# google-research/simclr

Hardware: AMD Instinct MI355X
Metric: images/sec (whole node), ResNet-50 1x SimCLR pretraining step @224px (higher is better)
Workload: dtype f32; 1 GPU; ResNet-50 1x, 224x224, 2 views/image, per-GPU batch 512, global batch 512, NT-Xent T=0.1 + linear-eval head + LARS, global BN, dp1; global_batch=512, parallelism=dp1

## Files before the change

simclr_amd/csrc/conv.hip:

```cpp
#include "common.h"
#include <stdlib.h>
#include <string.h>
#include <mutex>
#include <type_traits>

namespace {

enum { MODE_FWD = 0, MODE_DGRAD = 1 };

struct ConvP {
  const void* x;
  const void* w;
  void* y;
  float* stats;
  int V, IH, IW, IC, OH, OW, N, KH, KW, stride, pad;
  int pixpitch;
  int M, K;
  int nslot, accumulate;
  int m_tiles, n_tiles;
  int cs, py, px, cls_h, cls_w;
  int ntaps;
  int taps[9];
  unsigned long long tap_w, dy_w, dx_w;
  const void* bn_x;
// ... 30 lines not shown
template <> struct MMA<uint16_t> {
  __device__ static __forceinline__ f32x4 run(const u32x4& a, const u32x4& b, f32x4 c) {
    return __builtin_amdgcn_mfma_f32_16x16x32_bf16(__builtin_bit_cast(bf16x8, a),
                                                   __builtin_bit_cast(bf16x8, b), c, 0, 0, 0);
  }
};
template <> struct MMA<float> {
  __device__ static __forceinline__ f32x4 run(const u32x4& a, const u32x4& b, f32x4 c) {
#pragma unroll
    for (int j = 0; j < 4; ++j)
      c = __builtin_amdgcn_mfma_f32_16x16x4f32(__uint_as_float(a[j]), __uint_as_float(b[j]), c, 0, 0, 0);
    return c;
  }
};

__device__ __forceinline__ void split_terms2(const u32x4& c0, const u32x4& c1, u32x4& hi, u32x4& lo) {
#pragma unroll
  for (int j = 0; j < 4; ++j) {
    const float x0 = __uint_as_float(j < 2 ? c0[2 * j] : c1[2 * j - 4]), x1 = __uint_as_float(j < 2 ? c0[2 * j + 1] : c1[2 * j - 3]);
    const uint32_t h = pack_bf16x2(x0, x1);
    hi[j] = h;
    lo[j] = pack_bf16x2(x0 - __uint_as_float(h << 16), x1 - __uint_as_float(h & 0xffff0000u));
  }
}
__device__ __forceinline__ void split_terms3(const u32x4& c0, const u32x4& c1, u32x4& hi, u32x4& lo, u32x4& lo2) {
#pragma unroll
  for (int j = 0; j < 4; ++j) {
    const float x0 = __uint_as_float(j < 2 ? c0[2 * j] : c1[2 * j - 4]), x1 = __uint_as_float(j < 2 ? c0[2 * j + 1] : c1[2 * j - 3]);
    const uint32_t h = pack_bf16x2(x0, x1);
    const float r0 = x0 - __uint_as_float(h << 16), r1 = x1 - __uint_as_float(h & 0xffff0000u);
    const uint32_t l = pack_bf16x2(r0, r1);
    hi[j] = h;
    lo[j] = l;
    lo2[j] = pack_bf16x2(r0 - __uint_as_float(l << 16), r1 - __uint_as_float(l & 0xffff0000u));
  }
}
__device__ __forceinline__ f32x4 mma_bf16(const u32x4& a, const u32x4& b, f32x4 c) {
  return __builtin_amdgcn_mfma_f32_16x16x32_bf16(__builtin_bit_cast(bf16x8, a), __builtin_bit_cast(bf16x8, b), c, 0, 0, 0);
}
typedef __attribute__((ext_vector_type(8))) _Float16 f16x8;
#define F16_WSCALE_LOG2 8
__device__ __forceinline__ void split_terms2_f16(const u32x4& c0, const u32x4& c1, u32x4& hi, u32x4& lo) {
#pragma unroll
  for (int j = 0; j < 4; ++j) {
    const float x0 = __uint_as_float(j < 2 ? c0[2 * j] : c1[2 * j - 4]), x1 = __uint_as_float(j < 2 ? c0[2 * j + 1] : c1[2 * j - 3]);
    uint32_t h, l;
    split_pair<true>(x0, x1, h, l);
    hi[j] = h; lo[j] = l;
  }
}
__device__ __forceinline__ f32x4 mma_f16(const u32x4& a, const u32x4& b, f32x4 c) {
  return __builtin_amdgcn_mfma_f32_16x16x32_f16(__builtin_bit_cast(f16x8, a), __builtin_bit_cast(f16x8, b), c, 0, 0, 0);
}
template <int NA, int NB, bool TR, int terms, bool PSA = false, bool PSB2 = false, typename LA, typename LB>
__device__ __forceinline__ void mma_f32_chunks(f32x4* __restrict__ accp, LA lda, LB ldb) {
  static_assert(terms == 0 || terms == 3 || terms == 6 || terms == 13, "0 = exact fp32, 3 / 6 = split-bf16 terms, 13 = three split-fp16 terms");
  static_assert(!(PSA || PSB2) || terms == 3 || terms == 13, "pre-split operand: two planes (hi, lo) = the three-term products only");
#define acc_(i, j) accp[TR ? (j) * NA + (i) : (i) * NB + (j)]
  if constexpr (terms == 0) {
#pragma unroll
    for (int ks = 0; ks < 2; ++ks) {
      u32x4 a[NA], b[NB];
#pragma unroll
      for (int i = 0; i < NA; ++i) a[i] = lda(i, ks);
#pragma unroll
      for (int j = 0; j < NB; ++j) b[j] = ldb(j, ks);
#pragma unroll
      for (int i = 0; i < NA; ++i)
#pragma unroll
        for (int j = 0; j < NB; ++j)
#pragma unroll
          for (int e = 0; e < 4; ++e)
            acc_(i, j) = __builtin_amdgcn_mfma_f32_16x16x4f32(__uint_as_float(a[i][e]), __uint_as_float(b[j][e]), acc_(i, j), 0, 0, 0);
    }
  } else if constexpr (terms == 3 || terms == 13) {
    constexpr bool F16 = terms == 13;
    auto mm = [](const u32x4& a, const u32x4& b, f32x4 c) __attribute__((always_inline)) { return F16 ? mma_f16(a, b, c) : mma_bf16(a, b, c); };
    u32x4 bh[NB], bl[NB];
#pragma unroll
    for (int j = 0; j < NB; ++j) {
      if constexpr (PSB2) { bh[j] = ldb(j, 0); bl[j] = ldb(j, 1); }
      else if constexpr (F16) split_terms2_f16(ldb(j, 0), ldb(j, 1), bh[j], bl[j]);
      else split_terms2(ldb(j, 0), ldb(j, 1), bh[j], bl[j]);
    }
#pragma unroll
    for (int i = 0; i < NA; ++i) {
      u32x4 ah, al;
      if constexpr (PSA) { ah = lda(i, 0); al = lda(i, 1); }
      else if constexpr (F16) split_terms2_f16(lda(i, 0), lda(i, 1), ah, al);
      else split_terms2(lda(i, 0), lda(i, 1), ah, al);
#pragma unroll
      for (int j = 0; j < NB; ++j) acc_(i, j) = mm(al, bh[j], acc_(i, j));
#pragma unroll
      for (int j = 0; j < NB; ++j) acc_(i, j) = mm(ah, bl[j], acc_(i, j));
#pragma unroll
      for (int j = 0; j < NB; ++j) acc_(i, j) = mm(ah, bh[j], acc_(i, j));
    }
  } else {
    u32x4 bh[NB], bl[NB], bm[NB];
#pragma unroll
    for (int j = 0; j < NB; ++j) split_terms3(ldb(j, 0), ldb(j, 1), bh[j], bl[j], bm[j]);
#pragma unroll
    for (int i = 0; i < NA; ++i) {
      u32x4 ah, al, am;
      split_terms3(lda(i, 0), lda(i, 1), ah, al, am);
#pragma unroll
      for (int j = 0; j < NB; ++j) acc_(i, j) = mma_bf16(al, bl[j], acc_(i, j));
#pragma unroll
      for (int j = 0; j < NB; ++j) acc_(i, j) = mma_bf16(am, bh[j], acc_(i, j));
#pragma unroll
      for (int j = 0; j < NB; ++j) acc_(i, j) = mma_bf16(ah, bm[j], acc_(i, j));
#pragma unroll
      for (int j = 0; j < NB; ++j) acc_(i, j) = mma_bf16(al, bh[j], acc_(i, j));
#pragma unroll
      for (int j = 0; j < NB; ++j) acc_(i, j) = mma_bf16(ah, bl[j], acc_(i, j));
#pragma unroll
      for (int j = 0; j < NB; ++j) acc_(i, j) = mma_bf16(ah, bh[j], acc_(i, j));
    }
  }
#undef acc_
}

__device__ __forceinline__ u32x4 ld16(const void* p) { return *(const u32x4*)p; }
__device__ __forceinline__ u32x4 zero16() { return (u32x4){0u, 0u, 0u, 0u}; }

__device__ __forceinline__ bool tile_of_block(int m_tiles, int n_tiles, int& mt, int& nt) {
  const int b = blockIdx.x, xcd = b & 7, idx = b >> 3;
  nt = idx % n_tiles;
  mt = (idx / n_tiles) * 8 + xcd;
  return mt < m_tiles;
// ... 227 lines not shown
    constexpr int LPR = BN * 2 / 8;
    unsigned char* Cs = smem;
    long long* rowoff = (long long*)(smem + BM * PITCH);
    if (tid < BM) rowoff[tid] = row_offset(m0 + tid);
#pragma unroll
    for (int ni = 0; ni < NI; ++ni) {
      const int nl = wn * 64 + ni * 16 + g * 4;
#pragma unroll
      for (int mi = 0; mi < MI; ++mi) {
        const int ml = wm * (MI * 16) + mi * 16 + fl;
        u32x2 pk;
        pk[0] = pack_bf16x2(acc[ni][mi][0], acc[ni][mi][1]);
        pk[1] = pack_bf16x2(acc[ni][mi][2], acc[ni][mi][3]);
        *(u32x2*)(Cs + ml * PITCH + nl * 2) = pk;
      }
    }
    __syncthreads();
    const int c8 = tid % LPR;
    const int ncol = n0 + c8 * 4;
#pragma unroll 4
    for (int r = tid / LPR; r < BM; r += 256 / LPR) {
      const long long off = rowoff[r];
      if (off >= 0 && ncol < p.N) {
        u32x2 v = *(const u32x2*)(Cs + r * PITCH + c8 * 8);
        uint16_t* dst = (uint16_t*)Y + off + ncol;
        if (p.accumulate) {
          const u32x2 o = *(const u32x2*)dst;
          v[0] = pack_bf16x2(__uint_as_float(v[0] << 16) + __uint_as_float(o[0] << 16),
                             __uint_as_float(v[0] & 0xffff0000u) + __uint_as_float(o[0] & 0xffff0000u));
          v[1] = pack_bf16x2(__uint_as_float(v[1] << 16) + __uint_as_float(o[1] << 16),
                             __uint_as_float(v[1] & 0xffff0000u) + __uint_as_float(o[1] & 0xffff0000u));
        }
        *(u32x2*)dst = v;
      }
    }
  } else {
#pragma unroll
    for (int mi = 0; mi < MI; ++mi) {
      const long long off = row_offset(m0 + wm * (MI * 16) + mi * 16 + fl);
#pragma unroll
      for (int ni = 0; ni < NI; ++ni) {
        const int n = n0 + wn * 64 + ni * 16 + g * 4;
        if (off >= 0 && n < p.N) {
          T* dst = Y + off + n;
          float v[4] = {acc[ni][mi][0], acc[ni][mi][1], acc[ni][mi][2], acc[ni][mi][3]};
          if (p.accumulate) {
#pragma unroll
            for (int r = 0; r < 4; ++r) v[r] += Elem<T>::ld(dst + r);
          }
          *(float4*)dst = make_float4(v[0], v[1], v[2], v[3]);
        }
      }
    }
  }
}

#ifndef SIMCLR_BN64_WPE
#define SIMCLR_BN64_WPE 3
#endif
template <typename T, int MODE, int BM, int BN, int NW, int STAGES, bool STATS, bool BNEPI, bool EXT = false,
          bool WIN = false, bool FAPPLY = false, int SPL = 0, bool TAIL = false, bool PSB = false, int FAS = 0, int EPS = 0, bool PSX = false>
__global__ __launch_bounds__(NW * 64, (NW == 8 || STAGES == 3) ? 1 : (BN == 64 && (sizeof(T) == 2 || SPL == 13 || (SPL == 3 && PSB))) ? SIMCLR_BN64_WPE : 2) void conv_igemm_persistent(const ConvP p) {
  static_assert(EPS == 0 || (BNEPI && EPS <= 4 && (sizeof(T) == 2 || (MODE == MODE_DGRAD && SPL == 3 && PSB && PSX && !EXT))), "EPS specialises the BNEPI epilogue");
  const int bnm = EPS ? (((EPS - 1) >> 1) ? 4 : 2) : p.bn_mode;
  const bool accu = EPS ? ((EPS - 1) & 1) != 0 : p.accumulate != 0;
  static_assert(FAS == 0 || FAPPLY, "FAS specialises the FAPPLY epilogue");
  const bool fa_res = FAS ? true : p.bn_x != nullptr;
  const bool fa_rbn = FAS ? FAS == 2 : p.bn_mean != nullptr;
  const bool fa_relu = FAS ? true : p.bn_mode != 0;
  const bool fa_mask = FAS ? true : p.bn_mask != nullptr;
  const bool fa_n32 = FAS ? true : (p.N & 31) == 0;
  static_assert(!PSB || ((SPL == 3 || SPL == 13) && sizeof(T) == 4), "pre-split weights: fp32 storage, three terms");
  static_assert(!PSX || ((SPL == 3 || SPL == 13) && sizeof(T) == 4), "pre-split gathered operand: fp32 storage, three terms");
  static_assert(SPL != 13 || PSB, "split-fp16 terms need the pre-split (scaled) weight planes");
  static_assert(!WIN || (STAGES == 2 && !EXT && NW == 4 && BM == 128 && !FAPPLY && (sizeof(T) == 2 || ((SPL == 3 || SPL == 13) && PSB))),
                "halo-window variant: 2 stages; bf16, or fp32 storage with three terms and pre-split weights");
  static_assert(!FAPPLY || (MODE == MODE_FWD && !STATS && !BNEPI && !EXT), "fused BN-apply epilogue: forward, no statistics");
  static_assert(SPL == 0 || sizeof(T) == 4, "split-bf16 terms: fp32 storage only");
  constexpr bool WPS = WIN && sizeof(T) == 4 && !PSX && (SPL == 3 || SPL == 13);
  constexpr int EPC = Elem<T>::EPC;
  constexpr int BK = 8 * EPC;
  constexpr int WN = BN / 64;
  constexpr int WM = NW / WN;
  constexpr int MI = BM / WM / 16;
  constexpr int NI = 4;
  constexpr int AJ = BM / (8 * NW);
  constexpr int BJ = BN / (8 * NW);
  static_assert(AJ >= 1 && BJ >= 1 && MI >= 1, "tile / wave configuration");
  extern __shared__ __attribute__((aligned(16))) unsigned char smem[];
  constexpr int STG = (BM + BN) * 8;
  u32x4* As = (u32x4*)smem;
  u32x4* Bs = As + BM * 8;
  u32x4* Wn = (u32x4*)smem;
  u32x4* Bw = (u32x4*)(smem + (WIN ? p.win_bytes : 0));
  float* bnp = WIN ? (float*)(Bw + 2 * BN * 8)
                   : (float*)(As + STAGES * STG);
  long long* rowoff = (long long*)(bnp + (4 + (EXT ? 1 : 0)) * BN);
  const int zrow = WIN ? (int)(((unsigned char*)(rowoff + BM) - smem) >> 7) : 0;
  constexpr bool WSUM = BM == 256;
  float2* wred = (float2*)(rowoff + BM);
  constexpr bool LDS_EPI = sizeof(T) == 2;
  constexpr int NTH = NW * 64;
  constexpr int CPR = BN / 8;
  constexpr int RPP = NTH / CPR;
  constexpr bool ROWSTATS = STATS && LDS_EPI && (BNEPI || BM == 256);
  constexpr int EH = (LDS_EPI && BM * BN * 2 > STG * 16) ? 2 : 1;
// ... 72 lines not shown
    }
  };
  const T* b_src[BJ];
  bool b_ok[BJ];
#pragma unroll
  for (int j = 0; j < BJ; ++j) {
    const int n = n0 + 8 * (wave * BJ + j) + (lane >> 3);
    b_ok[j] = n < p.N;
    b_src[j] = Wt + (long long)(b_ok[j] ? n : 0) * p.K + kc * EPC;
  }
  auto issue_tile = [&](int ti, int ci, int buf) __attribute__((always_inline)) {
    if (DIAG(2)) return;
    const int ci0 = ci * BK;
    const bool ext = EXT && ti == p.ntaps;
    const int k0 = ext ? kmain + ci0 : (int)((p.tap_w >> (4 * ti)) & 15) * p.IC + ci0;
    unsigned char* a_dst = (unsigned char*)(As + buf * STG) + wave * AJ * 1024;
    unsigned char* b_dst = (unsigned char*)(Bs + buf * STG) + wave * BJ * 1024;
#pragma unroll
    for (int j = 0; j < AJ; ++j) {
      const void* src;
      if (ext) src = a_ok[j] ? (const void*)(X2 + (long long)a_m[j] * p.pixpitch2 + kc * EPC + ci0) : p.zero;
      else src = a_tok[j] ? (const void*)(a_tp[j] + ci0) : p.zero;
      __builtin_amdgcn_global_load_lds((gptr_t)src, (lptr_t)(a_dst + j * 1024), 16, 0, 0);
    }
#pragma unroll
    for (int j = 0; j < BJ; ++j) {
      const void* src = b_ok[j] ? (const void*)(b_src[j] + k0) : p.zero;
      __builtin_amdgcn_global_load_lds((gptr_t)src, (lptr_t)(b_dst + j * 1024), 16, 0, 0);
    }
  };

  if (BNEPI || EXT || FAPPLY) {
    for (int i = tid; i < BN; i += NW * 64) {
      const int n = n0 + i;
      const bool ok = n < p.N;
      if (FAPPLY) {
        bnp[i] = ok ? p.bn_scale[n] : 0.f;
        bnp[BN + i] = ok ? p.bn_shift[n] : 0.f;
        bnp[2 * BN + i] = (ok && p.bn_mean) ? p.bn_mean[n] : 1.f;
        bnp[3 * BN + i] = (ok && p.bn_rstd) ? p.bn_rstd[n] : 0.f;
      }
      if (BNEPI) {
        bnp[i] = (ok && bnm == 2) ? p.bn_scale[n] : 0.f;
        bnp[BN + i] = (ok && bnm == 2) ? p.bn_shift[n] : 0.f;
        bnp[2 * BN + i] = (ok && p.bn_mean) ? p.bn_mean[n] : 0.f;
        bnp[3 * BN + i] = (ok && p.bn_rstd) ? p.bn_rstd[n] : 0.f;
      }
      if (EXT) bnp[4 * BN + i] = (ok && p.bias) ? p.bias[n] : 0.f;
    }
  }
  if (WSUM && STATS && LDS_EPI) {
    for (int i = lane; i < BN; i += 64) wred[wave * BN + i] = make_float2(0.f, 0.f);
  }
  const int e_cc = tid % CPR;
  float e_s[8], e_q[8];
#pragma unroll
  for (int e = 0; e < 8; ++e) { e_s[e] = 0.f; e_q[e] = 0.f; }
  float st_s[NI][4], st_q[NI][4];
  if (STATS) {
#pragma unroll
    for (int i = 0; i < NI; ++i)
#pragma unroll
      for (int r = 0; r < 4; ++r) { st_s[i][r] = 0.f; st_q[i][r] = 0.f; }
  }

  int it = 0, iti = 0, ici = 0, ibuf = 0, buf = 0;
  int issued = 0, consumed = 0;
  const int KU = WIN ? kpt : KT;
  auto part_begin = [&]() __attribute__((always_inline)) { return (part_index() * KU) / p.rem_parts; };
  auto part_end = [&]() __attribute__((always_inline)) { return ((part_index() + 1) * KU) / p.rem_parts; };
  const int part_units = has_part ? part_end() - part_begin() : 0;
  const int total = WIN ? (count * kpt + part_units) * 9 : count * KT + part_units;
  auto issue_next = [&]() __attribute__((always_inline)) {
    issue_tile(iti, ici, ibuf);
    ibuf = (ibuf + 1 == STAGES) ? 0 : ibuf + 1;
    ++issued;
    if (++ici == ((EXT && iti == p.ntaps) ? kpt2 : kpt)) {
      ici = 0;
      if (++iti == p.ntaps + ((EXT && kpt2 > 0) ? 1 : 0)) {
        iti = 0;
        ++it;
        if (it < count) setup_rows(mslot + it * mslots);
        else if (it == count && has_part) {
          setup_rows(part_tile());
          const int pka = part_begin();
          iti = pka / kpt; ici = pka - iti * kpt;
          if (EXT && iti > p.ntaps) { iti = p.ntaps; ici = pka - p.ntaps * kpt; }
        }
      }
      if (it < count + (has_part ? 1 : 0) && iti < p.ntaps) set_tap(iti);
    }
  };
  const int Wd = p.IW;
  int wti = 0, wci = (WIN && count == 0 && has_part) ? part_begin() : 0, wit = 0;
  auto issue_b = [&]() __attribute__((always_inline)) {
    const int k0 = (int)((p.tap_w >> (4 * wti)) & 15) * p.IC + wci * BK;
    unsigned char* b_dst = (unsigned char*)(Bw + ibuf * (BN * 8)) + wave * BJ * 1024;
#pragma unroll
    for (int j = 0; j < BJ; ++j) {
      const void* src = b_ok[j] ? (const void*)(b_src[j] + k0) : p.zero;
      __builtin_amdgcn_global_load_lds((gptr_t)src, (lptr_t)(b_dst + j * 1024), 16, 0, 0);
    }
    ibuf ^= 1;
    ++issued;
    if (++wti == 9) {
      wti = 0;
// ... 79 lines not shown
        win_rows(t, zr, rr);
        if constexpr (sizeof(T) == 4) {
          mma_f32_chunks<NI, MI, false, SPL, PSB, PSX || WPS>(&acc[0][0],
              [&](int i, int ks) { const int r = wn * 64 + i * 16 + fl; return Bt[r * 8 + ((ks * 4 + g) ^ (r & 7))]; },
              [&](int i, int ks) { return Wc[rr[i] * 8 + ((ks * 4 + g) ^ (rr[i] & 7))]; });
        } else {
#pragma unroll
        for (int ks = 0; ks < 2; ++ks) {
          u32x4 af[MI], bf[NI];
          win_load(Wc, rr, Bt, ks, af, bf);
          win_mma(af, bf);
        }
        }
      };
      for (int c = kt0; c < kt1; ++c) {
        __syncthreads();
        issue_win(m0w, c);
        for (int t = 0; t < 9; ++t) {
          asm volatile("s_waitcnt vmcnt(0)" ::: "memory");
          __syncthreads();
          if (issued < total) issue_b();
          if constexpr (WPS) {
            if (t == 0) {
              const int nq = p.win_j * 32 * 4;
              for (int q = tid; q < nq; q += NW * 64) {
                const int row = q >> 2, gq = q & 3;
                u32x4* w0 = Wn + row * 8 + (gq ^ (row & 7));
                u32x4* w1 = Wn + row * 8 + ((4 + gq) ^ (row & 7));
                u32x4 hi, lo;
                if constexpr (SPL == 13) split_terms2_f16(*w0, *w1, hi, lo); else split_terms2(*w0, *w1, hi, lo);
                *w0 = hi; *w1 = lo;
              }
              __syncthreads();
            }
          }
          win_step(Wn, zrow, Bw + buf * (BN * 8), t);
          buf ^= 1;
          ++consumed;
        }
      }
    } else
    for (int kt = kt0; kt < kt1; ++kt) {
      if (STAGES == 3 && issued - consumed >= 2) asm volatile("s_waitcnt vmcnt(%0)" ::"n"(AJ + BJ) : "memory");
      else asm volatile("s_waitcnt vmcnt(0)" ::: "memory");
      if (STAGES == 3) {
        asm volatile("s_waitcnt lgkmcnt(0)" ::: "memory");
        __builtin_amdgcn_s_barrier();
      } else {
        __syncthreads();
      }
      if (issued < total) issue_next();
      if constexpr (sizeof(T) == 4) {
        if (!DIAG(1))
          mma_f32_chunks<NI, MI, false, SPL, PSB, PSX>(&acc[0][0],
              [&](int i, int ks) { const int r = wn * 64 + i * 16 + fl; return Bs[buf * STG + r * 8 + ((ks * 4 + g) ^ (r & 7))]; },
              [&](int i, int ks) { const int r = wm * (MI * 16) + i * 16 + fl; return As[buf * STG + r * 8 + ((ks * 4 + g) ^ (r & 7))]; });
      } else
      if (!DIAG(1))
#pragma unroll
      for (int ks = 0; ks < 2; ++ks) {
        constexpr int MH = MI > 4 ? 4 : MI;
        u32x4 bf[NI];
#pragma unroll
        for (int i = 0; i < NI; ++i) {
          const int r = wn * 64 + i * 16 + fl;
          bf[i] = Bs[buf * STG + r * 8 + ((ks * 4 + g) ^ (r & 7))];
        }
#pragma unroll
        for (int mh = 0; mh < MI; mh += MH) {
          u32x4 af[MH];
#pragma unroll
          for (int i = 0; i < MH; ++i) {
            const int r = wm * (MI * 16) + (mh + i) * 16 + fl;
            af[i] = As[buf * STG + r * 8 + ((ks * 4 + g) ^ (r & 7))];
          }
#pragma unroll
          for (int ni = 0; ni < NI; ++ni)
#pragma unroll
            for (int mi = 0; mi < MH; ++mi) acc[ni][mh + mi] = MMA<T>::run(bf[ni], af[mi], acc[ni][mh + mi]);
        }
      }
      buf = (buf + 1 == STAGES) ? 0 : buf + 1;
      ++consumed;
    }
    if (DIAG(4)) {
      if (acc[0][0][0] == 12345.678f) Y[0] = (T)0;
      continue;
    }
    if constexpr (SPL == 13) {
#pragma unroll
      for (int i = 0; i < NI; ++i)
#pragma unroll
        for (int j = 0; j < MI; ++j) acc[i][j] *= (1.0f / (float)(1 << F16_WSCALE_LOG2));
    }
    if (part) {
      const long long slot0 = ((long long)(mslot / p.rem_parts) * p.n_tiles + nt) * (p.rem_parts - 1);
      const int pj = part_index();
      constexpr int FR = NI * MI;
      if (pj != 0) {
        const __amdgpu_buffer_rsrc_t rp = __builtin_amdgcn_make_buffer_rsrc(
            (void*)((f32x4*)p.part_ws + (slot0 + pj - 1) * (long long)(FR * NTH)), 0, FR * NTH * 16, 0x00020000);
#pragma unroll
        for (int ni = 0; ni < NI; ++ni)
#pragma unroll
          for (int mi = 0; mi < MI; ++mi)
            __builtin_amdgcn_raw_buffer_store_b128(__builtin_bit_cast(u32x4, acc[ni][mi]), rp, tid * 16, (ni * MI + mi) * NTH * 16, 16);
        asm volatile("s_waitcnt vmcnt(0)" ::: "memory");
// ... 271 lines not shown
    auto load_row = [&](int mi) __attribute__((always_inline)) {
      const bool ok = offs[mi] >= 0;
      const long long a = ok ? offs[mi] : 0;
#pragma unroll
      for (int ni = 0; ni < NI; ++ni) {
        if (EAC) pr[ni] = *(const float4*)(Y + a + ni * 16);
        if (EBM == 2) xr[ni] = *(const float4*)(bx + a + ni * 16);
      }
      if (EBM == 4) mr = *(const u32x4*)(bmk + ((a - (ok ? g * 4 : 0)) >> 2));
    };
    load_row(0);
#pragma unroll
    for (int mi = 0; mi < MI; ++mi) {
#pragma unroll
      for (int ni = 0; ni < NI; ++ni) {
        if (offs[mi] >= 0) {
          const int nl = nl0 + ni * 16;
          float v[4] = {acc[ni][mi][0], acc[ni][mi][1], acc[ni][mi][2], acc[ni][mi][3]};
          if (EAC) { v[0] += pr[ni].x; v[1] += pr[ni].y; v[2] += pr[ni].z; v[3] += pr[ni].w; }
          float xf[4] = {0.f, 0.f, 0.f, 0.f}, mk[4];
          if (EBM == 4) {
            const unsigned mbits = mr[ni] >> (8 * g);
#pragma unroll
            for (int r = 0; r < 4; ++r) mk[r] = ((mbits >> r) & 1u) ? 1.f : 0.f;
          } else {
            xf[0] = xr[ni].x; xf[1] = xr[ni].y; xf[2] = xr[ni].z; xf[3] = xr[ni].w;
            const float4 sc = *(const float4*)(bnp + nl), sh = *(const float4*)(bnp + BN + nl);
            mk[0] = fmaf(xf[0], sc.x, sh.x); mk[1] = fmaf(xf[1], sc.y, sh.y);
            mk[2] = fmaf(xf[2], sc.z, sh.z); mk[3] = fmaf(xf[3], sc.w, sh.w);
          }
          const float4 mu = *(const float4*)(bnp + 2 * BN + nl), rs = *(const float4*)(bnp + 3 * BN + nl);
          const float mua[4] = {mu.x, mu.y, mu.z, mu.w}, rsa[4] = {rs.x, rs.y, rs.z, rs.w};
#pragma unroll
          for (int r = 0; r < 4; ++r) {
#pragma clang fp contract(off)
            v[r] = mk[r] > 0.f ? v[r] : 0.f;
            st_s[ni][r] += v[r];
            st_q[ni][r] += v[r] * (xf[r] - mua[r]) * rsa[r];
            acc[ni][mi][r] = v[r];
          }
        }
        __builtin_amdgcn_sched_barrier(0);
      }
      if (mi + 1 < MI) load_row(mi + 1);
      __builtin_amdgcn_sched_barrier(0);
      if (offs[mi] >= 0) {
#pragma unroll
        for (int ni = 0; ni < NI; ++ni)
          *(float4*)(Y + offs[mi] + ni * 16) = make_float4(acc[ni][mi][0], acc[ni][mi][1], acc[ni][mi][2], acc[ni][mi][3]);
      }
    }
    } else {
    float4 pvt[NI];
    if (sizeof(T) == 4 && MODE == MODE_FWD && STATS && !BNEPI && p.pivot) {
#pragma unroll
      for (int ni = 0; ni < NI; ++ni) {
        const int n = n0 + wn * 64 + ni * 16 + g * 4;
        pvt[ni] = n < p.N ? *(const float4*)(p.pivot + n) : make_float4(0.f, 0.f, 0.f, 0.f);
      }
    }
#pragma unroll
    for (int mi = 0; mi < MI; ++mi) {
      const int m = m0 + wm * (MI * 16) + mi * 16 + fl;
      long long off = -1;
      bool prior = p.accumulate != 0;
      if (flat) {
        if (m < p.M) off = (long long)m * p.N;
        if (p.accumulate == 2) {
          const int rem = m % (p.OH * p.OW), iy = rem / p.OW, ix = rem - iy * p.OW;
          prior = ((iy | ix) & 1) == 0;
        }
      } else if (m < p.M) {
        const int v = m / cls_hw;
        const int rem = m - v * cls_hw;
        const int ca = rem / p.cls_w, cb = rem - ca * p.cls_w;
        off = (((long long)v * p.OH + ca * p.cs + p.py) * p.OW + cb * p.cs + p.px) * p.N;
        if (p.accumulate == 2) prior = (((ca * p.cs + p.py) | (cb * p.cs + p.px)) & 1) == 0;
      }
#pragma unroll
      for (int ni = 0; ni < NI; ++ni) {
        const int n = n0 + wn * 64 + ni * 16 + g * 4;
        if (STATS && !BNEPI) {
          if (sizeof(T) == 4 && MODE == MODE_FWD && p.pivot) {
            if (off >= 0 && n < p.N) {
              const float pa[4] = {pvt[ni].x, pvt[ni].y, pvt[ni].z, pvt[ni].w};
#pragma unroll
              for (int r = 0; r < 4; ++r) { const float v = acc[ni][mi][r] - pa[r]; st_s[ni][r] += v; st_q[ni][r] += v * v; }
            }
          } else {
#pragma unroll
          for (int r = 0; r < 4; ++r) { const float v = acc[ni][mi][r]; st_s[ni][r] += v; st_q[ni][r] += v * v; }
          }
        }
        if (off >= 0 && n < p.N) {
          T* dst = Y + off + n;
          float v[4] = {acc[ni][mi][0], acc[ni][mi][1], acc[ni][mi][2], acc[ni][mi][3]};
          if (EXT) {
            const float4 bi = *(const float4*)(bnp + 4 * BN + wn * 64 + ni * 16 + g * 4);
            v[0] += bi.x; v[1] += bi.y; v[2] += bi.z; v[3] += bi.w;
          }
          if (prior) {
#pragma unroll
            for (int r = 0; r < 4; ++r) v[r] += Elem<T>::ld(dst + r);
          }
          if (BNEPI) {
            const int nl = wn * 64 + ni * 16 + g * 4;
            float xf[4] = {0.f, 0.f, 0.f, 0.f}, mk[4];
            if (p.bn_mode == 4) {
            } else if (sizeof(T) == 4) {
              const float4 xv = *(const float4*)((const float*)p.bn_x + off + n);
              xf[0] = xv.x; xf[1] = xv.y; xf[2] = xv.z; xf[3] = xv.w;
            } else {
              const u32x2 xv = *(const u32x2*)((const uint16_t*)p.bn_x + off + n);
              xf[0] = __uint_as_float(xv[0] << 16); xf[1] = __uint_as_float(xv[0] & 0xffff0000u);
              xf[2] = __uint_as_float(xv[1] << 16); xf[3] = __uint_as_float(xv[1] & 0xffff0000u);
            }
            if (p.bn_mode >= 3) {
              const unsigned mb = ((const unsigned char*)p.bn_mask)[(off + n) / EPC] >> (n % EPC);
#pragma unroll
              for (int r = 0; r < 4; ++r) mk[r] = ((mb >> r) & 1u) ? 1.f : 0.f;
            } else if (p.bn_mode == 1) {
              if (sizeof(T) == 4) {
                const float4 mv = *(const float4*)((const float*)p.bn_mask + off + n);
                mk[0] = mv.x; mk[1] = mv.y; mk[2] = mv.z; mk[3] = mv.w;
              } else {
                const u32x2 mv = *(const u32x2*)((const uint16_t*)p.bn_mask + off + n);
                mk[0] = __uint_as_float(mv[0] << 16); mk[1] = __uint_as_float(mv[0] & 0xffff0000u);
                mk[2] = __uint_as_float(mv[1] << 16); mk[3] = __uint_as_float(mv[1] & 0xffff0000u);
              }
            } else {
              const float4 sc = *(const float4*)(bnp + nl), sh = *(const float4*)(bnp + BN + nl);
              mk[0] = fmaf(xf[0], sc.x, sh.x); mk[1] = fmaf(xf[1], sc.y, sh.y);
              mk[2] = fmaf(xf[2], sc.z, sh.z); mk[3] = fmaf(xf[3], sc.w, sh.w);
            }
            const float4 mu = *(const float4*)(bnp + 2 * BN + nl), rs = *(const float4*)(bnp + 3 * BN + nl);
            const float mua[4] = {mu.x, mu.y, mu.z, mu.w}, rsa[4] = {rs.x, rs.y, rs.z, rs.w};
#pragma unroll
            for (int r = 0; r < 4; ++r) {
              v[r] = mk[r] > 0.f ? v[r] : 0.f;
              st_s[ni][r] += v[r];
              st_q[ni][r] += v[r] * (xf[r] - mua[r]) * rsa[r];
            }
          }
          if (sizeof(T) == 4) {
            *(float4*)dst = make_float4(v[0], v[1], v[2], v[3]);
          } else {
            u32x2 pk; pk[0] = pack_bf16x2(v[0], v[1]); pk[1] = pack_bf16x2(v[2], v[3]);
            *(u32x2*)dst = pk;
          }
        }
      }
    }
    }
  }
  if (ROWSTATS) {
    __syncthreads();
    float* red = WSUM ? (float*)wred : (float*)smem;
    constexpr int NRED = WSUM ? NW : RPP;
    if (!WSUM) {
#pragma unroll
      for (int e = 0; e < 8; ++e) {
        red[((tid / CPR) * BN + e_cc * 8 + e) * 2] = e_s[e];
        red[((tid / CPR) * BN + e_cc * 8 + e) * 2 + 1] = e_q[e];
      }
      __syncthreads();
    }
    const bool own_slot = p.nslot >= mslots;
    if (tid < BN && n0 + tid < p.N && (count > 0 || own_slot)) {
      float s1 = 0.f, s2 = 0.f;
      for (int w = 0; w < NRED; ++w) { s1 += red[(w * BN + tid) * 2]; s2 += red[(w * BN + tid) * 2 + 1]; }
      if (BNEPI) s2 = (s2 - bnp[2 * BN + tid] * s1) * bnp[3 * BN + tid];
      float* st = p.stats + (long long)(own_slot ? mslot : mslot % p.nslot) * 2 * p.N;
      if (own_slot) { st[n0 + tid] = s1; st[p.N + n0 + tid] = s2; }
      else { atomicAdd(st + n0 + tid, s1); atomicAdd(st + p.N + n0 + tid, s2); }
    }
    return;
  }
  if (STATS) {
    __syncthreads();
    float* red = (float*)smem;
#pragma unroll
    for (int ni = 0; ni < NI; ++ni) {
#pragma unroll
      for (int r = 0; r < 4; ++r) {
        float s = st_s[ni][r], ss = st_q[ni][r];
#pragma unroll
        for (int o = 1; o < 16; o <<= 1) { s += __shfl_xor(s, o, 64); ss += __shfl_xor(ss, o, 64); }
        if (fl == 0) {
          const int nl = wn * 64 + ni * 16 + g * 4 + r;
          red[(wm * BN + nl) * 2] = s;
          red[(wm * BN + nl) * 2 + 1] = ss;
        }
      }
    }
    __syncthreads();
    const bool own_slot = p.nslot >= mslots;
    if (tid < BN && n0 + tid < p.N && (count > 0 || own_slot)) {
      float s = 0.f, ss = 0.f;
#pragma unroll
      for (int w = 0; w < WM; ++w) { s += red[(w * BN + tid) * 2]; ss += red[(w * BN + tid) * 2 + 1]; }
      float* st = p.stats + (long long)(own_slot ? mslot : mslot % p.nslot) * 2 * p.N;
      if (own_slot) { st[n0 + tid] = s; st[p.N + n0 + tid] = ss; }
      else { atomicAdd(st + n0 + tid, s); atomicAdd(st + p.N + n0 + tid, ss); }
    }
  }
}

#include "igemm_wide.h"
#include "igemm_nwalk.h"

struct WgradP {
  const void* x;
  const void* dy;
  float* dw;
  int V, IH, IW, IC, OH, OW, N, KH, KW, stride, pad, pixpitch;
  int M, K, splits, chunks_per_split;
  int k_tiles, n_tiles;
  int xcd_map;
  const void* zero;
  int diag;
  int split;
  int dy_ps;
};

typedef __attribute__((ext_vector_type(4))) short s16x4_t;
typedef __attribute__((address_space(3))) s16x4_t lds_s16x4_t;

// ... 1632 lines not shown
  snprintf(name, sizeof(name), "conv_wgrad3x3_bf16<%d>", ST);
  record_wgrad(name, 2, "wgrad", grid, block, lds, rec_of(q));
  if (!dry_run()) hipLaunchKernelGGL(conv_wgrad3x3_bf16<ST>, dim3(grid), dim3(block), lds, stream, q);
}
static void run_wgrad3x3_f32ps(unsigned grid, unsigned block, size_t lds, hipStream_t stream, const Wgrad3P& q) {
  record_wgrad("conv_wgrad3x3_f32ps", 4, "wgrad", grid, block, lds, rec_of(q));
  if (!dry_run()) hipLaunchKernelGGL(conv_wgrad3x3_f32ps, dim3(grid), dim3(block), lds, stream, q);
}
template <int STAGES> static void run_stem_wgrad_ps(unsigned grid, unsigned block, size_t lds, hipStream_t stream, const StemWgP& p) {
  char name[64];
  snprintf(name, sizeof(name), "stem_wgrad_ps<7, 2, %d>", STAGES);
  record_wgrad(name, 4, "stem_wgrad_ps", grid, block, lds, rec_of(p));
  if (!dry_run()) hipLaunchKernelGGL((stem_wgrad_ps<7, 2, STAGES>), dim3(grid), dim3(block), lds, stream, p);
}
static void run_slab_reduce(const void* slabs, int splits, long long numel, float* out, int accumulate, hipStream_t stream) {
  const int grid = max(1, (int)ceil_div(numel / 4, 16));
  const size_t len = strlen(g_last_inst);
  snprintf(g_last_inst + len, sizeof(g_last_inst) - len, " reduce_grid=%d", grid);
  if (!dry_run()) hipLaunchKernelGGL(slab_reduce, dim3(grid), dim3(256), 0, stream, (const float*)slabs, splits, numel, out, accumulate);
}

static const void* zero_page() {
  static void* zp = nullptr;
  if (dry_run()) return (const void*)&g_last_inst;
  if (!zp && hipGetSymbolAddress(&zp, HIP_SYMBOL(g_zero16)) != hipSuccess) zp = nullptr;
  return zp;
}

static void igemm_persistent_grid(long long M, int N, int* bn, int* n_tiles, int* grid, bool narrow = false) {
  const int BN = (N <= 64 || narrow) ? 64 : 128;
  const int m_tiles = (int)((M + 127) / 128);
  const int nt = ceil_div(N, BN);
  const int unit = 8 * nt;
  const int resident = (BN == 64 ? 3 : 2) * 256;
  int pg = (resident / unit) * unit;
  if (pg < unit) pg = unit;
  const int need = ceil_div(m_tiles, 8) * unit;
  if (pg > need) pg = need;
  *bn = BN; *n_tiles = nt; *grid = pg;
}

static bool igemm_use_256(const ConvP& p, bool fwd) {
  if (p.N % 256 != 0 || p.ntaps <= 0 || p.N / 256 > 32) return false;
  const char* e = getenv("SIMCLR_IGEMM_TILE");
  const int mode = e ? atoi(e) : 0;
  if (mode == 256) return true;
  if (mode == 128) return false;
  if (p.KH != 1 || p.KW != 1 || p.M < 150000) return false;
  if (p.bn_mode && !p.fapply) return false;
  if (fwd && !p.fapply && p.stats && p.K < 128) return false;
  return !p.fapply;
}

static bool f32_epi_batch() {
  const char* e = getenv("SIMCLR_F32_EPI_BATCH");
  return !e || atoi(e) != 0;
}

static constexpr bool f32_eps_exists(bool win, int eps) { return !win && (eps == 1 || eps == 4); }

static bool igemm_use_wide(const ConvP& p, bool fwd) {
  const char* e = getenv("SIMCLR_IGEMM_WIDE");
  const int mode = e ? atoi(e) : 1;
  if (mode == 0) return false;
  if (p.N % 256 != 0 || p.N / 256 > 32 || p.ntaps <= 0 || p.IC % 64 != 0 || p.x2 || p.fapply) return false;
  if (p.bn_mode && p.bn_mode != 4 && !p.bn_x) return false;
  if ((long long)p.V * p.IH * p.IW * p.pixpitch * 2 >= 0xE0000000ll || (long long)p.N * p.K * 2 >= 0xE0000000ll) return false;
  if (mode == 2) return true;
  if (p.M < 32768) return false;
  if (fwd) return !(p.KH == 3 && p.KW == 3 && p.stride == 1) && 2.0 * (double)p.M * p.K * p.N >= 3.0e11;
  return !p.bn_mode && !p.accumulate && p.KH == 1 && p.KW == 1 && p.IC >= 512;
}

static bool igemm_narrow(const ConvP& p, size_t esz, bool dgrad = false) {
  constexpr int kmax = 64;
  constexpr int kmax32 = 128;
  if (esz == 4)
    return dgrad && p.split == 3 && p.N > 64 && p.KH == 1 && p.KW == 1 && p.stride == 1 && !p.x2 && p.K <= kmax32 && p.N / 64 <= 64;
  return esz == 2 && p.N > 64 && p.KH == 1 && p.KW == 1 && p.stride == 1 && !p.x2 && p.K <= kmax && p.N / 64 <= 64;
}

static std::mutex g_scratch_mutex;

struct SplitScratch { hipStream_t stream; float* ws; size_t floats; unsigned* flags; size_t nflags; };
static SplitScratch g_split_scratch[8];
static int g_split_scratch_n = 0;

static thread_local int g_last_split_parts = 0;
static void split_tail_plan(ConvP& p, int grid, int units, int unit_steps, bool wide = false) {
  p.rem_parts = 0; p.rem_full = 0; p.rem_tiles = 0; p.part_ws = nullptr; p.part_flags = nullptr; p.part_err = nullptr;
  const char* e = getenv("SIMCLR_IGEMM_SPLIT");
  const int mode = e ? atoi(e) : (wide ? 1 : 0);
  if (mode == 0 || p.n_tiles <= 0 || grid % p.n_tiles != 0) return;
  const int mslots = grid / p.n_tiles;
  const int full = p.m_tiles / mslots, R = p.m_tiles - full * mslots;
  const int max_parts = mode > 1 ? mode : 8;
  int P = R > 0 ? mslots / R : 0;
  if (P > max_parts) P = max_parts;
  constexpr int min_steps = 8;
  int max_parts_u = (units * unit_steps) / (min_steps > 0 ? min_steps : 1);
  if (max_parts_u > units) max_parts_u = units;
  if (P > max_parts_u) P = max_parts_u;
  if (R == 0 || full == 0 || P < 2 || full > 24) return;
  p.rem_full = full; p.rem_tiles = R; p.rem_parts = P;
}

// ... 179 lines not shown
    k.grid = min(max(unit, (256 / unit) * unit), ceil_div(p.m_tiles, 8) * unit);
    k.block = 512;
    k.tile_floats = (size_t)256 * 256;
    if (wide) {
      k.family = IgemmPlan::WIDE;
      p.x_bytes = (unsigned)((long long)p.V * p.IH * p.IW * p.pixpitch * 2);
      const int dist[3] = {8, 128, 136}, chw = p.cls_h * p.cls_w;
      for (int i = 0; i < 3; ++i) {
        p.rs_dq[i] = dist[i] / chw;
        const int r = dist[i] - p.rs_dq[i] * chw;
        p.rs_drow[i] = r / p.cls_w; p.rs_dcol[i] = r - p.rs_drow[i] * p.cls_w;
      }
      k.lds = 131072 + 4 * 256 * sizeof(float) + 256 * sizeof(long long) + 8 * 256 * 2 * sizeof(float) + 4 * 512 * sizeof(int);
      if (can_split) split_tail_plan(p, k.grid, p.ntaps * (p.IC / 64), 1, true);
      k.flat = p.KH == 1 && p.KW == 1 && p.stride == 1 && p.pad == 0 && p.cs == 1 && p.IH == p.OH && p.IW == p.OW;
    } else {
      k.family = IgemmPlan::TILE256;
      k.bn = 256;
      k.lds = 2 * (256 + 256) * 128 + 5 * 256 * sizeof(float) + 256 * sizeof(long long) + 8 * 256 * 2 * sizeof(float);
      k.fapply = p.fapply != 0;
      if (k.fapply) k.stats = k.bnepi = k.ext = false;
      else if (can_split) split_tail_plan(p, k.grid, p.ntaps * (p.IC / 64) + (p.x2 ? p.ic2 / 64 : 0), 1);
      k.tail = p.rem_parts >= 2;
    }
    return k;
  }
  k.family = IgemmPlan::TILE128;
  k.bn = BN;
  int pg, bn_, nt_;
  igemm_persistent_grid(p.M, p.N, &bn_, &nt_, &pg, narrow);
  k.grid = pg; k.block = 256;
  k.lds = 2 * (128 + BN) * 128 + 5 * BN * sizeof(float) + 128 * sizeof(long long);
  const bool win3 = (bf16 || p.split == 3 || p.split == 13) && !p.fapply && !p.x2 && p.KH == 3 && p.KW == 3 && p.stride == 1 &&
                    p.pad == 1 && p.cs == 1 && p.ntaps == 9 && p.IH == p.OH && p.IW == p.OW && p.IW <= 62 && p.accumulate < 2;
  const int bk_elems = 128 / (int)sizeof(T);
  if (bf16 && BN == 128 && !p.fapply && can_split) {
    split_tail_plan(p, pg, win3 ? p.IC / bk_elems : p.ntaps * (p.IC / bk_elems) + (p.x2 ? p.ic2 / bk_elems : 0), win3 ? 9 : 1);
    k.tile_floats = (size_t)128 * BN;
  } else {
    p.rem_parts = 0;
  }
  k.tail = p.rem_parts >= 2;
  if (!bf16) {
    const bool presplit = can_presplit && presplit_enabled(p.N, p.K);
    if (!fwd && p.split == 3) { k.psb = true; k.presplit = !p.w_ps && presplit; }
    if (fwd && p.split == 13) { k.psb = true; k.presplit = !p.w_ps && presplit; }
    if (k.psb && !p.w_ps && !presplit) {
      k.psb = false;
      if (fwd) p.split = 6;
    }
    if ((p.x_ps && !k.psb) || (p.w_ps && !k.psb)) { k.family = IgemmPlan::UNSUPPORTED; return k; }
    k.spl = k.psb || p.split == 3 || p.split == 6 ? p.split : 0;
    k.psx = k.psb && p.x_ps;
  }
  if (p.fapply) {
    k.fapply = true;
    k.stats = k.bnepi = k.ext = false;
    if (bf16 && p.bn_x && p.bn_mode && p.bn_mask && (p.N & 31) == 0) k.fas = p.bn_mean ? 2 : 1;
    if (!bf16 && fwd) plan_nwalk(k);
    return k;
  }
  int eps = 0;
  if (bf16 && !fwd && p.bn_mode && !k.tail) {
    if (p.bn_mode == 2 && !p.accumulate) eps = 1;
    else if (p.bn_mode == 4) eps = p.accumulate ? 4 : 3;
  }
  k.win = bf16 ? win3 : win3 && k.psb && (fwd ? !p.bn_mode : p.x_ps && (p.bn_mode != 0) == st);
  if (!bf16 && !fwd && k.psb && k.spl == 3 && k.psx && !k.ext && (p.bn_mode == 2 || p.bn_mode == 4) && p.accumulate < 2 && (p.N & 63) == 0 &&
      ((uintptr_t)p.bn_mask & 15) == 0 && f32_eps_exists(k.win, 1 + (p.bn_mode == 4 ? 2 : 0) + p.accumulate) && f32_epi_batch())
    eps = 1 + (p.bn_mode == 4 ? 2 : 0) + p.accumulate;
  if (k.win) {
    const int rows = ((128 + 2 * (p.IW + 1)) + 31) / 32 * 32;
    p.win_j = rows / 32;
    p.win_bytes = (!bf16 || rows * 128 > 128 * BN * 2) ? rows * 128 : 128 * BN * 2;
    k.lds = (size_t)p.win_bytes + 2 * BN * 128 + 5 * BN * sizeof(float) + 128 * sizeof(long long) + 128;
    k.eps = (!bf16 || eps == 1) ? eps : 0;
  } else {
    k.eps = !bf16 || eps == 1 || (!k.ext && eps >= 3) ? eps : 0;
    if (k.psx && k.ext) k.family = IgemmPlan::UNSUPPORTED;
  }
  return k;
}

template <typename V, V... Vs> struct among {};
template <typename F> static bool with_consts(F&& f) { return f(); }
template <typename V, V... Vs, typename... Rest, typename F>
static bool with_consts(F&& f, among<V, Vs...>, V x, Rest... rest) {
  bool hit = false;
  (void)((x == Vs && (hit = with_consts([&](auto... c) { return f(std::integral_constant<V, Vs>{}, c...); }, rest...), true)) || ...);
  return hit;
}
using Bools = among<bool, false, true>;

static constexpr bool epilogue_exists(bool st, bool be, bool ex) { return (st || !be) && (!ex || st == be); }
static constexpr bool tile128_exists(bool bf16, bool fwd, int bn, bool st, bool be, bool ex, bool win, bool fa, int spl, bool tail,
                                     bool psb, int fas, int eps, bool psx) {
  if (fa)
    return fwd && !st && !be && !ex && !win && !tail && !eps && !psx && (bf16 ? spl == 0 && !psb : fas == 0 && psb == (spl == 13));
  if (fas || !epilogue_exists(st, be, ex) || (win && ex)) return false;
  if (bf16)
    return spl == 0 && !psb && !psx && (eps ? st && be && !tail && (eps == 1 || (!ex && !win && (eps == 3 || eps == 4))) : !tail || bn == 128);
  if (tail) return false;
  if (eps) return !fwd && st && be && psb && spl == 3 && !ex && psx && f32_eps_exists(win, eps);
  if (win) return psb && (fwd ? spl == 13 && !be && !psx : spl == 3 && psx);
  if (psx) return !fwd && !ex && psb && spl == 3;
  if (psb) return fwd ? spl == 13 && !be && !ex : spl == 3;
  return spl == 0 || spl == 3 || spl == 6;
}

template <typename T, int MODE>
static bool launch_plan(const IgemmPlan& k, hipStream_t s) {
  constexpr bool bf16 = sizeof(T) == 2, fwd = MODE == MODE_FWD;
  const dim3 g(k.grid), b(k.block);
  switch (k.family) {
    case IgemmPlan::FALLBACK:
      return with_consts([&](auto BN, auto ST) { run_igemm<T, MODE, BN, ST, true>(g, b, k.lds, s, k.p); return true; },
                         among<int, 64, 128>{}, k.bn, Bools{}, k.stats);
    case IgemmPlan::WIDE:
      if constexpr (bf16)
        return with_consts([&](auto ST, auto BE, auto FLAT) {
          if constexpr (!epilogue_exists(ST, BE, false)) return false;
          else { run_wide<MODE, ST, BE, FLAT>(g, b, k.lds, s, k.p); return true; }
        }, Bools{}, k.stats, Bools{}, k.bnepi, Bools{}, k.flat);
      return false;
    case IgemmPlan::TILE256:
      if constexpr (bf16)
        return with_consts([&](auto ST, auto BE, auto EX, auto FA, auto TAIL) {
          if constexpr (FA ? !(fwd && !ST && !BE && !EX && !TAIL) : !epilogue_exists(ST, BE, EX)) return false;
          else { run_persistent<T, MODE, 256, 256, 8, 2, ST, BE, EX, false, FA, 0, TAIL>(g, b, k.lds, s, k.p); return true; }
        }, Bools{}, k.stats, Bools{}, k.bnepi, Bools{}, k.ext, Bools{}, k.fapply, Bools{}, k.tail);
      return false;
    case IgemmPlan::TILE128: {
      using Spl = std::conditional_t<bf16, among<int, 0>, among<int, 0, 3, 6, 13>>;
      using FpBools = std::conditional_t<bf16, among<bool, false>, Bools>;
      using HBools = std::conditional_t<bf16, Bools, among<bool, false>>;
      using Fas = std::conditional_t<bf16, among<int, 0, 1, 2>, among<int, 0>>;
      using Eps = std::conditional_t<bf16, among<int, 0, 1, 3, 4>, among<int, 0>>;
      if constexpr (!bf16 && !fwd) {
        if (k.eps)
          return k.stats && k.bnepi && !k.ext && !k.win && !k.fapply && k.spl == 3 && !k.tail && k.psb && !k.fas && k.psx &&
                 with_consts([&](auto BN, auto EPS) {
                   static_assert(f32_eps_exists(false, EPS), "the list below = the epilogues f32_eps_exists names");
                   run_persistent<T, MODE, 128, BN, 4, 2, true, true, false, false, false, 3, false, true, 0, EPS, true>(g, b, k.lds, s, k.p);
                   return true;
                 }, among<int, 64, 128>{}, k.bn, among<int, 1, 4>{}, k.eps);
      }
      return with_consts([&](auto BN, auto ST, auto BE, auto EX, auto WIN, auto FA, auto SPL, auto TAIL, auto PSB, auto FAS, auto EPS, auto PSX) {
        if constexpr (!tile128_exists(bf16, fwd, BN, ST, BE, EX, WIN, FA, SPL, TAIL, PSB, FAS, EPS, PSX)) return false;
        else { run_persistent<T, MODE, 128, BN, 4, 2, ST, BE, EX, WIN, FA, SPL, TAIL, PSB, FAS, EPS, PSX>(g, b, k.lds, s, k.p); return true; }
      }, among<int, 64, 128>{}, k.bn, Bools{}, k.stats, Bools{}, k.bnepi, Bools{}, k.ext, Bools{}, k.win, Bools{}, k.fapply, Spl{}, k.spl,
         HBools{}, k.tail, FpBools{}, k.psb, Fas{}, k.fas, Eps{}, k.eps, FpBools{}, k.psx);
    }
    case IgemmPlan::NWALK:
      if constexpr (!bf16 && fwd)
        return with_consts([&](auto KPT, auto FAS) { run_nwalk<KPT, FAS>(g, b, k.lds, s, k.p); return true; },
                           among<int, 2, 4>{}, k.p.IC / 32, among<int, 1, 2>{}, k.fas);
      return false;
    default:
      return false;
  }
}

template <typename T, int MODE>
static int launch_igemm_one(const ConvP& p, hipStream_t stream) {
  bool can_split = true, can_presplit = true;
  IgemmPlan k = plan_igemm<T, MODE>(p, can_split, can_presplit);
  if (k.family == IgemmPlan::UNSUPPORTED) return 1;
  if (k.p.rem_parts >= 2 && !split_tail_scratch(k.p, k.tile_floats, stream)) k = plan_igemm<T, MODE>(p, can_split = false, can_presplit);
  if (k.presplit) {
    const void* ws = presplit_weights(k.p.w, k.p.N, k.p.K, stream, k.spl == 13);
    if (ws) k.p.w = ws;
    else k = plan_igemm<T, MODE>(p, can_split, can_presplit = false);
  }
  if (k.family == IgemmPlan::EMPTY) return 0;
  if (k.family == IgemmPlan::UNSUPPORTED) return 1;
  if (k.family != IgemmPlan::FALLBACK) g_last_split_parts = k.p.rem_parts;
  if (sizeof(T) == 4 && MODE == MODE_DGRAD && k.family == IgemmPlan::TILE128) g_last_presplit = k.psb;
  return launch_plan<T, MODE>(k, stream) ? 0 : 1;
}

template <typename T, int MODE>
static int launch_igemm(const ConvP& p0, hipStream_t stream) {
  ConvP p = p0;
  if (MODE == MODE_FWD || p.stride == 1) {
    p.cs = 1; p.py = 0; p.px = 0; p.cls_h = p.OH; p.cls_w = p.OW;
    p.ntaps = p.KH * p.KW;
    p.tap_w = p.dy_w = p.dx_w = 0;
    for (int t = 0; t < p.ntaps; ++t) {
      p.taps[t] = t;
      const int ty = t / p.KW, tx = t % p.KW;
      const int dy = (MODE == MODE_FWD) ? ty : p.pad - ty, dx = (MODE == MODE_FWD) ? tx : p.pad - tx;
      p.tap_w |= (unsigned long long)t << (4 * t);
      p.dy_w |= (unsigned long long)(dy + 8) << (4 * t);
      p.dx_w |= (unsigned long long)(dx + 8) << (4 * t);
    }
    p.M = p.V * p.OH * p.OW;
    return launch_igemm_one<T, MODE>(p, stream);
  }
  const int S = p.stride;
  ConvP cls[4];
  int n = 0;
  for (int py = 0; py < S; ++py)
    for (int px = 0; px < S; ++px) {
      ConvP q = p;
      q.cs = S; q.py = py; q.px = px;
      q.cls_h = (p.OH - py + S - 1) / S;
      q.cls_w = (p.OW - px + S - 1) / S;
      q.ntaps = 0;
      q.tap_w = q.dy_w = q.dx_w = 0;
      for (int ty = 0; ty < p.KH; ++ty)
        for (int tx = 0; tx < p.KW; ++tx)
          if ((py + p.pad - ty) % S == 0 && (px + p.pad - tx) % S == 0 && q.ntaps < 9) {
            q.tap_w |= (unsigned long long)(ty * p.KW + tx) << (4 * q.ntaps);
            q.dy_w |= (unsigned long long)((py + p.pad - ty) / S + 8) << (4 * q.ntaps);
            q.dx_w |= (unsigned long long)((px + p.pad - tx) / S + 8) << (4 * q.ntaps);
            q.taps[q.ntaps++] = ty * p.KW + tx;
          }
      q.M = p.V * q.cls_h * q.cls_w;
      if (q.ntaps == 0 && p.accumulate == 2 && ((py | px) & 1)) q.accumulate = 0;
      else if (q.ntaps == 0 && p.accumulate) continue;
      if (p.accumulate == 3) q.accumulate = 0;
      if (q.ntaps == 0) q.x_ps = 0;
      if (plan_igemm<T, MODE>(q, true, true).family == IgemmPlan::UNSUPPORTED) return 1;
      cls[n++] = q;
    }
  for (int i = 0; i < n; ++i)
    if (int rc = launch_igemm_one<T, MODE>(cls[i], stream)) return rc;
  return 0;
}

// ... 695 lines not shown
```

Measured before the change: 3742 images/s.

## Add 256x256 tile path for large fp32 split-precision 1x1 convolutions

Routes large 1x1 fp32 convolutions (forward with split-fp16 terms and stats, dgrad with pre-split bf16 operands) to a 256x256 tile, 8-wave persistent kernel when M is large enough relative to the slot count. The goal is more operand reuse per loaded tile and less global traffic. It adds a HOLDA MMA ordering that keeps the A fragments in registers while streaming B, so register pressure stays manageable at the larger tile. It also adds a shuffle-fold reduction of BN column statistics into LDS for this path. The risks are lower occupancy, register spills and load imbalance on layers near the threshold.

Result: no change. 3775 images/s (median of 6 runs) (+0.9%).

```diff
diff --git a/simclr_amd/csrc/conv.hip b/simclr_amd/csrc/conv.hip
--- a/simclr_amd/csrc/conv.hip
+++ b/simclr_amd/csrc/conv.hip
@@ -106,7 +106,7 @@
 __device__ __forceinline__ f32x4 mma_f16(const u32x4& a, const u32x4& b, f32x4 c) {
   return __builtin_amdgcn_mfma_f32_16x16x32_f16(__builtin_bit_cast(f16x8, a), __builtin_bit_cast(f16x8, b), c, 0, 0, 0);
 }
-template <int NA, int NB, bool TR, int terms, bool PSA = false, bool PSB2 = false, typename LA, typename LB>
+template <int NA, int NB, bool TR, int terms, bool PSA = false, bool PSB2 = false, bool HOLDA = false, typename LA, typename LB>
 __device__ __forceinline__ void mma_f32_chunks(f32x4* __restrict__ accp, LA lda, LB ldb) {
   static_assert(terms == 0 || terms == 3 || terms == 6 || terms == 13, "0 = exact fp32, 3 / 6 = split-bf16 terms, 13 = three split-fp16 terms");
   static_assert(!(PSA || PSB2) || terms == 3 || terms == 13, "pre-split operand: two planes (hi, lo) = the three-term products only");
@@ -130,6 +130,29 @@
   } else if constexpr (terms == 3 || terms == 13) {
     constexpr bool F16 = terms == 13;
     auto mm = [](const u32x4& a, const u32x4& b, f32x4 c) __attribute__((always_inline)) { return F16 ? mma_f16(a, b, c) : mma_bf16(a, b, c); };
+    if constexpr (HOLDA) {
+      u32x4 ah[NA], al[NA];
+#pragma unroll
+      for (int i = 0; i < NA; ++i) {
+        if constexpr (PSA) { ah[i] = lda(i, 0); al[i] = lda(i, 1); }
+        else if constexpr (F16) split_terms2_f16(lda(i, 0), lda(i, 1), ah[i], al[i]);
+        else split_terms2(lda(i, 0), lda(i, 1), ah[i], al[i]);
+      }
+#pragma unroll
+      for (int j = 0; j < NB; ++j) {
+        u32x4 bh, bl;
+        if constexpr (PSB2) { bh = ldb(j, 0); bl = ldb(j, 1); }
+        else if constexpr (F16) split_terms2_f16(ldb(j, 0), ldb(j, 1), bh, bl);
+        else split_terms2(ldb(j, 0), ldb(j, 1), bh, bl);
+#pragma unroll
+        for (int i = 0; i < NA; ++i) acc_(i, j) = mm(al[i], bh, acc_(i, j));
+#pragma unroll
+        for (int i = 0; i < NA; ++i) acc_(i, j) = mm(ah[i], bl, acc_(i, j));
+#pragma unroll
+        for (int i = 0; i < NA; ++i) acc_(i, j) = mm(ah[i], bh, acc_(i, j));
+      }
+      return;
+    }
     u32x4 bh[NB], bl[NB];
 #pragma unroll
     for (int j = 0; j < NB; ++j) {
@@ -463,6 +486,15 @@
         }
       }
     }
+  }
+}
+
+template <int H> __device__ __forceinline__ void fold16(float* v, int fl) {
+  const bool up = (fl & (H / 2)) != 0;
+#pragma unroll
+  for (int i = 0; i < H; ++i) {
+    const float keep = up ? v[i + H] : v[i], send = up ? v[i] : v[i + H];
+    v[i] = keep + __shfl_xor(send, H / 2, 64);
   }
 }
 
@@ -641,6 +673,11 @@
   if (WSUM && STATS && LDS_EPI) {
     for (int i = lane; i < BN; i += 64) wred[wave * BN + i] = make_float2(0.f, 0.f);
   }
+  constexpr bool TSUM = WSUM && STATS && !BNEPI && sizeof(T) == 4;
+  float* tsum = (float*)wred + wave * 128;
+  if (TSUM) {
+    tsum[lane] = 0.f; tsum[64 + lane] = 0.f;
+  }
   const int e_cc = tid % CPR;
   float e_s[8], e_q[8];
 #pragma unroll
@@ -826,7 +863,7 @@
       if (issued < total) issue_next();
       if constexpr (sizeof(T) == 4) {
         if (!DIAG(1))
-          mma_f32_chunks<NI, MI, false, SPL, PSB, PSX>(&acc[0][0],
+          mma_f32_chunks<NI, MI, false, SPL, PSB, PSX, BM == 256>(&acc[0][0],
               [&](int i, int ks) { const int r = wn * 64 + i * 16 + fl; return Bs[buf * STG + r * 8 + ((ks * 4 + g) ^ (r & 7))]; },
               [&](int i, int ks) { const int r = wm * (MI * 16) + i * 16 + fl; return As[buf * STG + r * 8 + ((ks * 4 + g) ^ (r & 7))]; });
       } else
@@ -1204,6 +1241,13 @@
     }
     } else {
     float4 pvt[NI];
+    float tv[TSUM ? 2 * NI * 4 : 1];
+    if (TSUM) {
+#pragma unroll
+      for (int i = 0; i < 2 * NI * 4; ++i) tv[i] = 0.f;
+    }
+    float (*us)[4] = TSUM ? (float (*)[4])&tv[0] : st_s;
+    float (*uq)[4] = TSUM ? (float (*)[4])&tv[TSUM ? NI * 4 : 0] : st_q;
     if (sizeof(T) == 4 && MODE == MODE_FWD && STATS && !BNEPI && p.pivot) {
 #pragma unroll
       for (int ni = 0; ni < NI; ++ni) {
@@ -1237,11 +1281,11 @@
             if (off >= 0 && n < p.N) {
               const float pa[4] = {pvt[ni].x, pvt[ni].y, pvt[ni].z, pvt[ni].w};
 #pragma unroll
-              for (int r = 0; r < 4; ++r) { const float v = acc[ni][mi][r] - pa[r]; st_s[ni][r] += v; st_q[ni][r] += v * v; }
+              for (int r = 0; r < 4; ++r) { const float v = acc[ni][mi][r] - pa[r]; us[ni][r] += v; uq[ni][r] += v * v; }
             }
           } else {
 #pragma unroll
-          for (int r = 0; r < 4; ++r) { const float v = acc[ni][mi][r]; st_s[ni][r] += v; st_q[ni][r] += v * v; }
+          for (int r = 0; r < 4; ++r) { const float v = acc[ni][mi][r]; us[ni][r] += v; uq[ni][r] += v * v; }
           }
         }
         if (off >= 0 && n < p.N) {
@@ -1303,6 +1347,12 @@
         }
       }
     }
+    if constexpr (TSUM) {
+      fold16<16>(tv, fl); fold16<8>(tv, fl); fold16<4>(tv, fl); fold16<2>(tv, fl);
+      const int col = ((fl >> 1) & 3) * 16 + g * 4 + 2 * (fl & 1);
+      float* dst = tsum + (fl >> 3) * 64 + col;
+      dst[0] += tv[0]; dst[1] += tv[1];
+    }
     }
   }
   if (ROWSTATS) {
@@ -1325,6 +1375,22 @@
       float* st = p.stats + (long long)(own_slot ? mslot : mslot % p.nslot) * 2 * p.N;
       if (own_slot) { st[n0 + tid] = s1; st[p.N + n0 + tid] = s2; }
       else { atomicAdd(st + n0 + tid, s1); atomicAdd(st + p.N + n0 + tid, s2); }
+    }
+    return;
+  }
+  if constexpr (TSUM) {
+    __syncthreads();
+    const bool own_slot = p.nslot >= mslots;
+    if (tid < BN && n0 + tid < p.N && (count > 0 || own_slot)) {
+      float s = 0.f, ss = 0.f;
+#pragma unroll
+      for (int w = 0; w < WM; ++w) {
+        const float* src = (const float*)wred + (w * WN + (tid >> 6)) * 128 + (tid & 63);
+        s += src[0]; ss += src[64];
+      }
+      float* st = p.stats + (long long)(own_slot ? mslot : mslot % p.nslot) * 2 * p.N;
+      if (own_slot) { st[n0 + tid] = s; st[p.N + n0 + tid] = ss; }
+      else { atomicAdd(st + n0 + tid, s); atomicAdd(st + p.N + n0 + tid, ss); }
     }
     return;
   }
@@ -3063,6 +3129,20 @@
   return !p.fapply;
 }
 
+static bool igemm_use_256_f32(const ConvP& p, bool fwd, bool psb, int spl, bool psx, bool stats, bool ext) {
+  if (p.N % 256 != 0 || p.N / 256 > 32 || p.ntaps != 1 || p.KH != 1 || p.KW != 1 || p.IC < 256 || p.IC % 32 != 0) return false;
+  if (p.fapply || p.bn_mode || ext || !psb) return false;
+  if (fwd ? !(spl == 13 && stats && !psx) : !(spl == 3 && psx && !stats)) return false;
+  const char* e = getenv("SIMCLR_IGEMM_TILE");
+  const int mode = e ? atoi(e) : 0;
+  if (mode == 256) return true;
+  if (mode == 128) return false;
+  if (p.M < 150000) return false;
+  const int n_tiles = p.N / 256, unit = 8 * n_tiles, m_tiles = ceil_div(p.M, 256);
+  const int mslots = min(max(unit, (256 / unit) * unit), ceil_div(m_tiles, 8) * unit) / n_tiles;
+  return m_tiles >= (fwd ? 6 : 12) * mslots;
+}
+
 static bool f32_epi_batch() {
   const char* e = getenv("SIMCLR_F32_EPI_BATCH");
   return !e || atoi(e) != 0;
@@ -3348,6 +3428,17 @@
     if ((p.x_ps && !k.psb) || (p.w_ps && !k.psb)) { k.family = IgemmPlan::UNSUPPORTED; return k; }
     k.spl = k.psb || p.split == 3 || p.split == 6 ? p.split : 0;
     k.psx = k.psb && p.x_ps;
+    if (igemm_use_256_f32(p, fwd, k.psb, k.spl, k.psx, k.stats, k.ext)) {
+      p.m_tiles = ceil_div(p.M, 256);
+      p.n_tiles = p.N / 256;
+      const int unit = 8 * p.n_tiles;
+      k.family = IgemmPlan::TILE256;
+      k.bn = 256;
+      k.grid = min(max(unit, (256 / unit) * unit), ceil_div(p.m_tiles, 8) * unit);
+      k.block = 512;
+      k.lds = 2 * (256 + 256) * 128 + 5 * 256 * sizeof(float) + 256 * sizeof(long long) + 8 * 256 * 2 * sizeof(float);
+      return k;
+    }
   }
   if (p.fapply) {
     k.fapply = true;
@@ -3425,7 +3516,17 @@
           if constexpr (FA ? !(fwd && !ST && !BE && !EX && !TAIL) : !epilogue_exists(ST, BE, EX)) return false;
           else { run_persistent<T, MODE, 256, 256, 8, 2, ST, BE, EX, false, FA, 0, TAIL>(g, b, k.lds, s, k.p); return true; }
         }, Bools{}, k.stats, Bools{}, k.bnepi, Bools{}, k.ext, Bools{}, k.fapply, Bools{}, k.tail);
-      return false;
+      else {
+        if (k.bnepi || k.ext || k.win || k.fapply || k.tail || !k.psb || k.fas || k.eps) return false;
+        if constexpr (fwd) {
+          if (k.spl != 13 || !k.stats || k.psx) return false;
+          run_persistent<T, MODE, 256, 256, 8, 2, true, false, false, false, false, 13, false, true>(g, b, k.lds, s, k.p);
+        } else {
+          if (k.spl != 3 || k.stats || !k.psx) return false;
+          run_persistent<T, MODE, 256, 256, 8, 2, false, false, false, false, false, 3, false, true, 0, 0, true>(g, b, k.lds, s, k.p);
+        }
+        return true;
+      }
     case IgemmPlan::TILE128: {
       using Spl = std::conditional_t<bf16, among<int, 0>, among<int, 0, 3, 6, 13>>;
       using FpBools = std::conditional_t<bf16, among<bool, false>, Bools>;
@@ -3471,7 +3572,7 @@
   if (k.family == IgemmPlan::EMPTY) return 0;
   if (k.family == IgemmPlan::UNSUPPORTED) return 1;
   if (k.family != IgemmPlan::FALLBACK) g_last_split_parts = k.p.rem_parts;
-  if (sizeof(T) == 4 && MODE == MODE_DGRAD && k.family == IgemmPlan::TILE128) g_last_presplit = k.psb;
+  if (sizeof(T) == 4 && MODE == MODE_DGRAD && (k.family == IgemmPlan::TILE128 || k.family == IgemmPlan::TILE256)) g_last_presplit = k.psb;
   return launch_plan<T, MODE>(k, stream) ? 0 : 1;
 }
 
```
